# kirilllzaitsev/vision_mtl

Hardware: AMD Instinct MI355X
Metric: images/sec fwd+bwd, basic model 128x256 (higher is better)
Workload: dtype f32

## Files before the change

### include/vmtl.h

```cpp
#ifndef VMTL_H
#define VMTL_H

#ifdef __cplusplus
extern "C" {
#endif

#define VMTL_ACT_NONE 0
#define VMTL_ACT_RELU 1
#define VMTL_ACT_HSWISH 2
#define VMTL_ACT_HSIGMOID 3
#define VMTL_ACT_SIGMOID 4

#define VMTL_PREC_FP32 0
#define VMTL_PREC_BF16 1

const char* vmtl_version(void);
const char* vmtl_last_error_string(void);
int vmtl_reload_env(void);
int vmtl_timestamp(long long* out, void* stream);


int vmtl_conv2d_fwd(const float* x, const float* wp, const float* bias, float* y, float* stats,
                    int B, int H, int W, int Cs, int Ho, int Wo, int ldy, int Nw, int Cout,
                    int KH, int KW, int stride, int pad, int act, int shuffle, void* stream);
int vmtl_conv2d_fwd_p(const float* x, const float* wp, const float* bias, float* y, float* stats,
                      int B, int H, int W, int Cs, int Ho, int Wo, int ldy, int Nw, int Cout,
                      int KH, int KW, int stride, int pad, int act, int shuffle, int precision, void* stream);
int vmtl_conv2d_ksplit(int B, int Ho, int Wo, int ldy, int Ktot);
int vmtl_conv2d_fwd_ws(const float* x, const float* wp, const float* bias, float* y, float* ws, int B, int H, int W, int Cs,
                       int Ho, int Wo, int ldy, int Nw, int Cout, int KH, int KW, int stride, int pad, void* stream);
int vmtl_conv2d_fwd_ws_p(const float* x, const float* wp, const float* bias, float* y, float* ws, int B, int H, int W,
                         int Cs, int Ho, int Wo, int ldy, int Nw, int Cout, int KH, int KW, int stride, int pad,
                         int precision, void* stream);
int vmtl_conv2d_stats_rows(int B, int Ho, int Wo, int ldy);
int vmtl_conv2d_stats_block(int B, int Ho, int Wo, int ldy);

int vmtl_conv1x1_stats_block(int M, int ldy, int Ks, int variant);
int vmtl_conv1x1_stats_rows(int M, int ldy, int Ks, int variant);
int vmtl_conv1x1_fwd(const float* x, const float* wp, const float* bias, float* y, float* stats, int M, int Ks, int ldy,
                     int Nw, int Cout, void* stream);
int vmtl_conv1x1_fwd_p(const float* x, const float* wp, const float* bias, float* y, float* stats, int M, int Ks, int ldy,
                       int Nw, int Cout, int precision, void* stream);
int vmtl_conv1x1_cat_fwd(const float* x, int K1, const float* x2, int K2s, const float* wp, const float* bias, float* y,
                         float* stats, int M, int ldy, int Nw, int Cout, void* stream);
int vmtl_conv1x1_cat_dgrad(const float* dy, const float* wp, float* dx, int N1, float* dx2, int N2s, int N2, int M,
                           int Ks, void* stream);
int vmtl_conv1x1_cat_fwd_p(const float* x, int K1, const float* x2, int K2s, const float* wp, const float* bias, float* y,
                           float* stats, int M, int ldy, int Nw, int Cout, int precision, void* stream);
int vmtl_conv1x1_cat_dgrad_p(const float* dy, const float* wp, float* dx, int N1, float* dx2, int N2s, int N2, int M,
                             int Ks, int precision, void* stream);
int vmtl_conv1x1_cat_wgrad(const float* x, int K1, const float* x2, int K2s, const float* dy, float* slabs, int splits,
                           int M, int ldy, int Nw, void* stream);
int vmtl_conv1x1_cat_wgrad_p(const float* x, int K1, const float* x2, int K2s, const float* dy, float* slabs, int splits,
                             int M, int ldy, int Nw, int precision, void* stream);
int vmtl_conv1x1_bn_fwd(const float* x, const float* coef_a, const float* coef_c, int act_in, float* a_out,
                        const float* wp, const float* bias, float* y, float* stats, int M, int Ks, int ldy, int Nw,
                        int Cout, void* stream);
int vmtl_conv1x1_bnbwd(const float* dy, const float* wp, float* dz, float* stats, const float* ez_x,
                       const float* ez_mean, const float* ez_invstd, const float* ez_gamma, const float* ez_beta,
                       int ez_act, int M, int Ks, int ldy, int Nw, int Cout, void* stream);
int vmtl_conv1x1_bn_fwd_p(const float* x, const float* coef_a, const float* coef_c, int act_in, float* a_out,
                          const float* wp, const float* bias, float* y, float* stats, int M, int Ks, int ldy, int Nw,
                          int Cout, int precision, void* stream);
int vmtl_conv1x1_bnbwd_p(const float* dy, const float* wp, float* dz, float* stats, const float* ez_x,
                         const float* ez_mean, const float* ez_invstd, const float* ez_gamma, const float* ez_beta,
                         int ez_act, int M, int Ks, int ldy, int Nw, int Cout, int precision, void* stream);
int vmtl_conv1x1_bn_res_fwd(const float* x, const float* coef_a, const float* coef_c, int act_in, const float* res,
                            float* a_out, const float* wp, const float* bias, float* y, float* stats, int M, int Ks,
                            int ldy, int Nw, int Cout, void* stream);
int vmtl_conv1x1_bnbwd_add(const float* dy, const float* wp, const float* addend, float* dz, float* stats,
                           const float* ez_x, const float* ez_mean, const float* ez_invstd, const float* ez_gamma,
                           const float* ez_beta, int ez_act, int M, int Ks, int ldy, int Nw, int Cout, void* stream);
int vmtl_conv1x1_bn_res_fwd_p(const float* x, const float* coef_a, const float* coef_c, int act_in, const float* res,
                              float* a_out, const float* wp, const float* bias, float* y, float* stats, int M, int Ks,
                              int ldy, int Nw, int Cout, int precision, void* stream);
int vmtl_conv1x1_bnbwd_add_p(const float* dy, const float* wp, const float* addend, float* dz, float* stats,
                             const float* ez_x, const float* ez_mean, const float* ez_invstd, const float* ez_gamma,
                             const float* ez_beta, int ez_act, int M, int Ks, int ldy, int Nw, int Cout, int precision,
                             void* stream);

int vmtl_conv2d_bnbwd(const float* x, const float* wp, float* y, float* stats, const float* ez_x, const float* ez_mean,
                      const float* ez_invstd, const float* ez_gamma, const float* ez_beta, int ez_act, int B, int H,
                      int W, int Cs, int Ho, int Wo, int ldy, int Nw, int Cout, int KH, int KW, int stride, int pad,
                      void* stream);
int vmtl_conv2d_bnbwd_p(const float* x, const float* wp, float* y, float* stats, const float* ez_x, const float* ez_mean,
                        const float* ez_invstd, const float* ez_gamma, const float* ez_beta, int ez_act, int B, int H,
                        int W, int Cs, int Ho, int Wo, int ldy, int Nw, int Cout, int KH, int KW, int stride, int pad,
                        int precision, void* stream);

int vmtl_conv2d_up2_fwd(const float* xl, const float* skip, const float* wp_eff, float* y, float* stats,
                        int B, int H2, int W2, int C0s, int C1s, int ldy, int Cout, void* stream);
int vmtl_conv2d_up2_fwd_p(const float* xl, const float* skip, const float* wp_eff, float* y, float* stats,
                          int B, int H2, int W2, int C0s, int C1s, int ldy, int Cout, int precision, void* stream);
int vmtl_conv2d_up2_stats_block(int B, int H2, int W2, int ldy);
int vmtl_conv2d_up2_ksplit(int B, int H2, int W2, int ldy, int Ktot);
int vmtl_conv2d_up2_fwd_ws(const float* xl, const float* skip, const float* wp_eff, float* y, float* ws, int B, int H2,
                           int W2, int C0s, int C1s, int ldy, int Cout, void* stream);
int vmtl_conv2d_up2_fwd_ws_p(const float* xl, const float* skip, const float* wp_eff, float* y, float* ws, int B, int H2,
                             int W2, int C0s, int C1s, int ldy, int Cout, int precision, void* stream);
int vmtl_conv2d_up2_halo(const float* xl, const float* skip, const float* wp_eff, float* y, float* stats,
                         int B, int H2, int W2, int C0s, int C1s, int ldy, int Cout, void* stream);
int vmtl_conv2d_up2_halo_supported(int B, int H2, int W2, int C0s, int C1s, int ldy, int Cout);
int vmtl_conv2d_up2_halo_stat_rows(int B, int H2, int W2, int C0s, int C1s, int ldy, int Cout);
int vmtl_conv2d_up2_halo_stat_block(int C0s, int C1s, int ldy, int Cout);
int vmtl_pack_up2_fwd(const float* w, float* dst, int Cout, int C0, int C0s, int C1, int C1s, void* stream);
int vmtl_pack_up2_dgrad(const float* w, float* dst, int Cout, int Cos, int C0, int Cin, void* stream);
int vmtl_unpack_up2(const float* slabs, float* grad, int Cout, int Cos, int C0, int Cin, int nslabs, void* stream);

int vmtl_conv2d_wgrad_splits(int M, int Nw, int Ktot);
int vmtl_conv2d_wgrad(const float* x, const float* dy, float* slabs, int splits, int B, int H, int W, int Cs,
                      int Ho, int Wo, int ldy, int Nw, int KH, int KW, int stride, int pad, void* stream);
int vmtl_conv2d_wgrad_p(const float* x, const float* dy, float* slabs, int splits, int B, int H, int W, int Cs,
                        int Ho, int Wo, int ldy, int Nw, int KH, int KW, int stride, int pad, int precision,
                        void* stream);

int vmtl_conv3x3_wgrad_small_supported(int Cs, int ldy, int W);
int vmtl_conv3x3_wgrad_small_slabs(int B, int H, int W);
int vmtl_conv3x3_wgrad_small(const float* x, const float* dy, float* slabs, int nslabs, int B, int H, int W, int Cs,
                             int ldy, int Nw, void* stream);


int vmtl_conv3x3_small_supported(int Cs, int Nw);
int vmtl_conv3x3_small_tiles(int B, int H, int W);
int vmtl_conv3x3_small_stat_rows(int B, int H, int W);
int vmtl_conv3x3_small_stat_block(int B, int H, int W);
int vmtl_conv3x3_small(const float* x, const float* x2, const float* pa, const float* pb, const float* pc,
                       int act_in, float* a_out, const float* wp, const float* bias, float* y, float* yb, int Ca,
                       float* stats, int ep_mode, const float* ez_x, const float* ez_mean, const float* ez_invstd,
                       const float* ez_gamma, const float* ez_beta, int ez_act, int B, int H, int W, int Cs, int ldy,
                       int Nw, int Cout, void* stream);

int vmtl_conv3x3_halo_supported(int B, int H, int W, int Cs, int ldy, int Nw);
int vmtl_conv3x3_halo_stat_rows(int B, int H, int W);
int vmtl_conv3x3_halo_stat_block(int B, int H, int W);
int vmtl_conv3x3_halo(const float* x, const float* pa, const float* pc, int act_in, float* a_out, const float* wp,
                      const float* bias, float* y, float* stats, int ep_mode, const float* ez_x, const float* ez_mean,
                      const float* ez_invstd, const float* ez_gamma, const float* ez_beta, int ez_act, int B, int H,
                      int W, int Cs, int ldy, int Nw, int Cout, void* stream);

int vmtl_dwconv_fwd(const float* x, const float* wp, float* y, int B, int H, int W, int Cs, int Ho, int Wo,
                    int K, int stride, int pad, void* stream);
int vmtl_dwconv_bn_stats_rows(int M, int Cs);
int vmtl_dwconv_bn_stats_block(int M, int Cs);
int vmtl_dwconv_bn_fwd(const float* x, const float* coef_a, const float* coef_c, int act, const float* wp, float* y,
                       float* a_out, float* partial, int B, int H, int W, int Cs, int Ho, int Wo, int K, int stride,
                       int pad, void* stream);
int vmtl_dwconv_bwd_data(const float* dy, const float* wp, float* dx, int B, int H, int W, int Cs, int Ho,
                         int Wo, int K, int stride, int pad, void* stream);
int vmtl_dwconv_bwd_data_add(const float* dy, const float* wp, const float* addend, float* dx, int B, int H, int W,
                             int Cs, int Ho, int Wo, int K, int stride, int pad, void* stream);
int vmtl_dwconv_bwd_weight_rows(int M, int Cs);
int vmtl_dwconv_bwd_weight(const float* x, const float* dy, float* partial, float* dw, int B, int H, int W,
                           int C, int Cs, int Ho, int Wo, int K, int stride, int pad, void* stream);
#define VMTL_DW_ROUTE_ACT_MASK 3
#define VMTL_DW_ROUTE_SPEC 4
#define VMTL_DW_ROUTE_K5 8
#define VMTL_DW_ROUTE_S2 16
#define VMTL_DW_ROUTE_WLDS 32
#define VMTL_DW_ROUTE_FIN32 64
#define VMTL_DW_ROUTE_QL(r) (1 << (((r) >> 8) & 7))
int vmtl_dwconv_bn_fwd_route(int B, int H, int W, int Cs, int Ho, int Wo, int K, int stride, int pad, int act);
int vmtl_dwconv_bwd_data_route(int B, int H, int W, int Cs, int Ho, int Wo, int K, int stride, int pad);
int vmtl_dwconv_bwd_weight_route(int B, int H, int W, int C, int Cs, int Ho, int Wo, int K, int stride, int pad);

int vmtl_pack_weights(const float* src, float* dst, int R1, int R0, int T, int C, int Cs, long long sr1,
                      long long sr0, long long st, long long sc, int flip, void* stream);
int vmtl_pack_weights_scaled(const float* src, float* dst, int R1, int R0, int T, int C, int Cs, long long sr1,
                             long long sr0, long long st, long long sc, int flip, const float* scale, int sstride,
                             int smode, void* stream);
int vmtl_unpack_weights_stitch(const float* packed, float* grad, const float* w, const float* scale, int sstride,
                               float* ds, float* work, int R0, int T, int C, int Cs, int nslabs, long long slab_stride,
                               int reduce_all, void* stream);
int vmtl_pack_desc_bytes(void);
int vmtl_pack_weights_batch(const void* descs, int n, long long total, void* stream);
int vmtl_pack_weights_slice(const float* src, float* dst, int R0, int T, int C, int group, long long sr0,
                            long long st, long long sc, int flip, void* stream);
int vmtl_unpack_weights(const float* packed, float* grad, int R1, int R0, int T, int C, int Cs,
                        long long sr1, long long sr0, long long st, long long sc, int flip, int nslabs,
                        long long slab_stride, void* stream);

int vmtl_reduce_rows(int M);
int vmtl_bn_stats(const float* x, int M, int C, int Cs, float* partial, int nblk_from_conv,
                  int rows_per_blk_from_conv, float eps, float momentum, float* running_mean, float* running_var, long long* num_batches_tracked,
                  float* save_mean, float* save_invstd, void* stream);
int vmtl_bn_eval_stats(const float* running_mean, const float* running_var, int C, int Cs, float eps,
                       float* save_mean, float* save_invstd, void* stream);
int vmtl_bn_stats_coef(const float* x, int M, int C, int Cs, float* partial, int nblk_from_conv,
                       int rows_per_blk_from_conv, float eps, float momentum, float* running_mean, float* running_var,
                       long long* num_batches_tracked, float* save_mean, float* save_invstd, const float* gamma,
                       const float* beta, float* coef_a, float* coef_c, void* stream);
int vmtl_bn_eval_stats_coef(const float* running_mean, const float* running_var, int C, int Cs, float eps,
                            float* save_mean, float* save_invstd, const float* gamma, const float* beta,
                            float* coef_a, float* coef_c, void* stream);
int vmtl_bn_eval_desc_bytes(void);
int vmtl_bn_eval_stats_batch(const void* descs, int n, int max_cs, void* stream);
int vmtl_bn_apply(const float* x, const float* mean, const float* invstd, const float* gamma,
                  const float* beta, const float* mul, const float* res, float* y, long long M, int C,
                  int Cs, int act, void* stream);
int vmtl_bn_fuse_max_rows(void);
int vmtl_bn_apply_fused(const float* x, const float* partial, int nblk, int rows_per_blk, float eps, float momentum,
                        float* running_mean, float* running_var, long long* num_batches_tracked, float* save_mean,
                        float* save_invstd, const float* gamma, const float* beta, const float* mul, const float* res,
                        float* y, long long M, int C, int Cs, int act, void* stream);
int vmtl_bn_bwd(const float* x, const float* dy, const float* mean, const float* invstd, const float* gamma,
                const float* beta, const float* mul, float* dmul, float* partial, float* sum_dz,
                float* sum_dzx, float* dx, int M, int C, int Cs, int act, int training, void* stream);
int vmtl_bn_bwd_finalize(const float* partial, int nblk, int M, int C, int Cs, float* sum_dz, float* sum_dzx,
                         const float* mean, const float* invstd, const float* gamma, int training, float* coef_a,
                         float* coef_b, float* coef_c, void* stream);
int vmtl_bn_bwd_apply(const float* x, const float* dz, const float* mean, const float* invstd, const float* gamma,
                      const float* sum_dz, const float* sum_dzx, float* dx, int M, int C, int Cs, int training,
                      void* stream);

int vmtl_bn_act_pool2_fwd(const float* x, const float* mean, const float* invstd, const float* gamma,
                          const float* beta, float* y, int B, int H, int W, int C, int Cs, int act, void* stream);
int vmtl_bn_act_pool2_bwd(const float* x, const float* dyp, const float* mean, const float* invstd,
                          const float* gamma, const float* beta, float* partial, float* sum_dz, float* sum_dzx,
                          float* dx, int B, int H, int W, int C, int Cs, int act, int training, void* stream);

int vmtl_conv2d_dgrad_s2_supported(int K, int pad);
long long vmtl_conv2d_dgrad_s2_ws(int B, int H, int W, int Cs, int Ho, int Wo, int ldy, int K, int pad);
long long vmtl_pack_dgrad_s2_size(int Cin, int ldy, int K, int pad);
int vmtl_pack_dgrad_s2(const float* w, float* dst, int Cout, int Cin, int ldy, int K, int pad, void* stream);
int vmtl_conv2d_dgrad_s2(const float* dy, const float* wp, float* dx, float* ws, int B, int H, int W, int Cs, int Ho,
                         int Wo, int ldy, int Cin, int K, int pad, void* stream);
int vmtl_conv2d_dgrad_s2_p(const float* dy, const float* wp, float* dx, float* ws, int B, int H, int W, int Cs, int Ho,
                           int Wo, int ldy, int Cin, int K, int pad, int precision, void* stream);
int vmtl_bn_act_pool3s2_fwd(const float* x, const float* mean, const float* invstd, const float* gamma,
                            const float* beta, float* a_out, float* y, unsigned char* idx, int B, int H, int W, int C,
                            int Cs, int act, void* stream);
int vmtl_bn_act_pool3s2_bwd(const float* x, const float* dskip, const float* dyp, const unsigned char* idx,
                            const float* mean, const float* invstd, const float* gamma, const float* beta, float* dz,
                            float* partial, float* sum_dz, float* sum_dzx, float* dx, int B, int H, int W, int C, int Cs,
                            int act, int training, void* stream);
int vmtl_bn_add_act_fwd(const float* z, const float* mean_a, const float* invstd_a, const float* gamma_a,
                        const float* beta_a, const float* res, const float* zd, const float* mean_b, const float* invstd_b,
                        const float* gamma_b, const float* beta_b, float* y, int M, int C, int Cs, int act, void* stream);
int vmtl_bn_add_act_bwd(const float* z, const float* mean_a, const float* invstd_a, const float* gamma_a,
                        const float* beta_a, const float* res, const float* zd, const float* mean_b, const float* invstd_b,
                        const float* gamma_b, const float* beta_b, const float* dy, float* g, float* partial,
                        float* sum_dz_a, float* sum_dzx_a, float* sum_dz_b, float* sum_dzx_b, float* dz, float* dzd, int M,
                        int C, int Cs, int act, int training, void* stream);

int vmtl_colsum(const float* a, const float* b, int M, int C, int Cs, int mode, int reduce_all,
                float* partial, float* out, void* stream);

int vmtl_concat2(const float* a, int Ha, int Wa, int Ca, int Csa, int upa, int oha, int owa,
                 const float* b, int Hb, int Wb, int Cb, int Csb, int upb, int ohb, int owb, float* y,
                 int B, int H, int W, int Cd, void* stream);
int vmtl_concat2_bwd(const float* dy, float* dx, int B, int H, int W, int Cd, int c_off, int Hs, int Ws,
                     int C, int Cs, int up, int oh, int ow, void* stream);
int vmtl_maxpool2_fwd(const float* x, float* y, int B, int H, int W, int Cs, void* stream);
int vmtl_maxpool2_bwd(const float* x, const float* dy, float* dx, int B, int H, int W, int Cs, void* stream);
int vmtl_bilinear_up2_fwd(const float* x, float* y, int B, int H, int W, int Cs, void* stream);
int vmtl_bilinear_up2_bwd(const float* dy, float* dx, int B, int H, int W, int Cs, void* stream);
int vmtl_spatial_mean(const float* x, float* y, int B, int HW, int Cs, void* stream);
int vmtl_channel_bcast(const float* x, const float* s, float* y, int B, int HW, int Cs, int mode, void* stream);
int vmtl_channel_scale_bwd_s(const float* x, const float* dy, float* ds, int B, int HW, int Cs, void* stream);
int vmtl_fc_max_rows(void);
int vmtl_fc_fwd(const float* a, int a_parts, long long a_part_stride, float a_scale, const float* a_z, int a_act,
                float* a_out, const float* w, const float* bias, float* z, float* y, int M, int K, int N, int lda,
                int ldw, int ldy, int act, void* stream);
int vmtl_fc_wgrad(const float* x, int x_parts, long long x_part_stride, float x_scale, const float* dyo, int dy_parts,
                  long long dy_part_stride, const float* zo, float* dw, float* db, int M, int K, int N, int lda, int ldn,
                  int act, void* stream);
int vmtl_hw_reduce_parts(int B, int HW, int Cs);
int vmtl_hw_reduce(const float* x, const float* y, float* part, int B, int HW, int Cs, void* stream);
int vmtl_channel_scale_add(const float* x, const float* s, const float* t, float t_scale, float* y, int B, int HW,
                           int Cs, void* stream);
int vmtl_se_gate_supported(int B, int C, int R);
// ... 159 lines not shown
```

### vision_mtl_amd/csrc/conv_wgrad_small.hip

```cpp
#include "common.h"

#define WS_SW 32
#define WS_LDP 48
#define WS_XROW ((WS_SW + 2) * WS_LDP)
#define WS_YROW (WS_SW * WS_LDP)

struct WsP {
  const float* x;
  const float* dy;
  float* slabs;
  int B, H, W, Cs, ldy, Nw, Ktot;
  int R;
  int bands, strips;
};

template <int NI, int JW>
__global__ __launch_bounds__(256) void wgrad_small_kernel(WsP p) {
  __shared__ __attribute__((aligned(16))) float Xs[4 * WS_XROW];
  __shared__ __attribute__((aligned(16))) float Ys[2 * WS_YROW];
  const int tid = threadIdx.x;
  const int lane = tid & 63, wn = tid >> 6;
  const int l15 = lane & 15, lq = lane >> 4;

  const int seg = blockIdx.x;
  const int band = seg % p.bands;
  const int t0 = seg / p.bands;
  const int strip = t0 % p.strips, b = t0 / p.strips;
  const int c0 = strip * WS_SW;
  const int r0 = band * p.R, r1 = min(p.H, r0 + p.R);

  for (int i = tid; i < (4 * WS_XROW) / 4; i += 256) reinterpret_cast<f32x4*>(Xs)[i] = (f32x4){0.f, 0.f, 0.f, 0.f};
  for (int i = tid; i < (2 * WS_YROW) / 4; i += 256) reinterpret_cast<f32x4*>(Ys)[i] = (f32x4){0.f, 0.f, 0.f, 0.f};

  const int CQ = p.Cs >> 2, YQ = p.ldy >> 2;
  constexpr unsigned OOB = 0xFFFFFFFFu;
  int xoff[2], xlds[2];
#pragma unroll
  for (int it = 0; it < 2; ++it) {
    const int idx = tid + it * 256;
    const int px = idx / CQ, q = idx - px * CQ;
    const int c = c0 - 1 + px;
    const bool ok = idx < (WS_SW + 2) * CQ && c >= 0 && c < p.W;
    xoff[it] = ok ? (c * p.Cs + q * 4) * 4 : -1;
    xlds[it] = idx < (WS_SW + 2) * CQ ? px * WS_LDP + q * 4 : -1;
  }
  int yoff[2], ylds[2];
#pragma unroll
  for (int it = 0; it < 2; ++it) {
    const int idx = tid + it * 256;
    const int px = idx / YQ, q = idx - px * YQ;
    const bool ok = idx < WS_SW * YQ;
    yoff[it] = ok ? ((c0 + px) * p.ldy + q * 4) * 4 : -1;
    ylds[it] = ok ? px * WS_LDP + q * 4 : -1;
  }
  const __amdgpu_buffer_rsrc_t rs_x =
      buf_rsrc(p.x, (int)((unsigned)p.B * p.H * p.W * p.Cs * 4u));
  const __amdgpu_buffer_rsrc_t rs_dy =
      buf_rsrc(p.dy, (int)((unsigned)p.B * p.H * p.W * p.ldy * 4u));
  auto load_x = [&](int rr, f32x4* rx) {
    const bool rok = rr >= 0 && rr < p.H;
    const unsigned base = (unsigned)(b * p.H + rr) * (unsigned)p.W * (unsigned)p.Cs * 4u;
#pragma unroll
    for (int it = 0; it < 2; ++it) rx[it] = buf_load16(rs_x, (rok & (xoff[it] >= 0)) ? base + (unsigned)xoff[it] : OOB);
  };
  auto load_y = [&](int rr, f32x4* ry) {
    const bool rok = rr < r1;
    const unsigned base = (unsigned)(b * p.H + rr) * (unsigned)p.W * (unsigned)p.ldy * 4u;
#pragma unroll
    for (int it = 0; it < 2; ++it) ry[it] = buf_load16(rs_dy, (rok & (yoff[it] >= 0)) ? base + (unsigned)yoff[it] : OOB);
  };
  auto store_x = [&](int rr, const f32x4* rx) {
    float* xs = Xs + ((rr + 1) & 3) * WS_XROW;
#pragma unroll
    for (int it = 0; it < 2; ++it)
      if (xlds[it] >= 0) *reinterpret_cast<f32x4*>(xs + xlds[it]) = rx[it];
  };
  auto store_y = [&](int buf, const f32x4* ry) {
    float* ys = Ys + buf * WS_YROW;
#pragma unroll
    for (int it = 0; it < 2; ++it)
      if (ylds[it] >= 0) *reinterpret_cast<f32x4*>(ys + ylds[it]) = ry[it];
  };

  int bdh[JW];
  int bcol[JW];
#pragma unroll
  for (int jw = 0; jw < JW; ++jw) {
    const int kk = (wn + 4 * jw) * 16 + l15;
    if (kk < p.Ktot) {
      const int tap = kk / p.Cs, ci = kk - tap * p.Cs;
      const int th = tap / 3;
      bdh[jw] = th - 1;
      bcol[jw] = (lq + tap - 3 * th) * WS_LDP + ci;
    } else {
      bdh[jw] = 0;
      bcol[jw] = lq * WS_LDP + p.Cs;
    }
  }
  const int acol = lq * WS_LDP + l15;

  f32x4 acc[NI][JW];
#pragma unroll
  for (int i = 0; i < NI; ++i)
#pragma unroll
    for (int jw = 0; jw < JW; ++jw) acc[i][jw] = (f32x4){0.f, 0.f, 0.f, 0.f};

  f32x4 rx[2], ry[2];
  __syncthreads();
  load_x(r0 - 1, rx);
  store_x(r0 - 1, rx);
  load_x(r0, rx);
  store_x(r0, rx);
  load_x(r0 + 1, rx);
  store_x(r0 + 1, rx);
  load_y(r0, ry);
  store_y(0, ry);
  __syncthreads();

  for (int r = r0; r < r1; ++r) {
    const int buf = (r - r0) & 1;
    const bool more = r + 1 < r1;
    if (more) {
      load_x(r + 2, rx);
      load_y(r + 1, ry);
    }
    const float* ys = Ys + buf * WS_YROW + acol;
    const float* xb[JW];
#pragma unroll
    for (int jw = 0; jw < JW; ++jw) xb[jw] = Xs + ((r + bdh[jw] + 1) & 3) * WS_XROW + bcol[jw];
#pragma unroll
    for (int s = 0; s < WS_SW / 4; ++s) {
      float fa[NI], fb[JW];
#pragma unroll
      for (int i = 0; i < NI; ++i) fa[i] = ys[4 * s * WS_LDP + i * 16];
#pragma unroll
      for (int jw = 0; jw < JW; ++jw) fb[jw] = xb[jw][4 * s * WS_LDP];
#pragma unroll
      for (int i = 0; i < NI; ++i)
#pragma unroll
        for (int jw = 0; jw < JW; ++jw)
          acc[i][jw] = __builtin_amdgcn_mfma_f32_16x16x4f32(fa[i], fb[jw], acc[i][jw], 0, 0, 0);
    }
    if (more) {
      store_x(r + 2, rx);
      store_y(buf ^ 1, ry);
    }
    __syncthreads();
  }

  float* slab = p.slabs + (size_t)seg * p.Nw * p.Ktot;
#pragma unroll
  for (int i = 0; i < NI; ++i)
#pragma unroll
    for (int jw = 0; jw < JW; ++jw) {
      const int kk = (wn + 4 * jw) * 16 + l15;
#pragma unroll
      for (int e = 0; e < 4; ++e) {
        const int co = i * 16 + 4 * lq + e;
        if (co < p.Nw && kk < p.Ktot) slab[(size_t)co * p.Ktot + kk] = acc[i][jw][e];
      }
    }
}

static void ws_geometry(int B, int H, int W, int* R, int* bands, int* strips) {
  static EnvInt e_target{"VMTL_WS_TARGET", 1024};
  const int st = W / WS_SW;
  long long nb = cdivll((long long)env_int(e_target), (long long)B * st);
  if (nb < 1) nb = 1;
  int rows = cdiv(H, (int)nb);
  if (rows < 8) rows = H < 8 ? H : 8;
  *R = rows;
  *bands = cdiv(H, rows);
  *strips = st;
}

extern "C" int vmtl_conv3x3_wgrad_small_supported(int Cs, int ldy, int W) {
  static EnvInt e{"VMTL_WGRAD_SMALL", 1};
  return env_int(e) != 0 && Cs >= 4 && Cs <= 36 && !(Cs & 3) && ldy >= 4 && ldy <= 36 && !(ldy & 3) && !(Cs > 32 && ldy > 32) &&
         W >= WS_SW && W % WS_SW == 0;
}

extern "C" int vmtl_conv3x3_wgrad_small_slabs(int B, int H, int W) {
  if (B <= 0 || H <= 0 || W < WS_SW || W % WS_SW) return 0;
  int R, bands, strips;
  ws_geometry(B, H, W, &R, &bands, &strips);
  return B * strips * bands;
}

template <int NI>
static int ws_launch(const WsP& p, int jwn, int grid, hipStream_t st) {
  switch (jwn) {
    case 1: hipLaunchKernelGGL((wgrad_small_kernel<NI, 1>), dim3(grid), dim3(256), 0, st, p); break;
    case 2: hipLaunchKernelGGL((wgrad_small_kernel<NI, 2>), dim3(grid), dim3(256), 0, st, p); break;
    case 3: hipLaunchKernelGGL((wgrad_small_kernel<NI, 3>), dim3(grid), dim3(256), 0, st, p); break;
    case 4: hipLaunchKernelGGL((wgrad_small_kernel<NI, 4>), dim3(grid), dim3(256), 0, st, p); break;
    case 5: hipLaunchKernelGGL((wgrad_small_kernel<NI, 5>), dim3(grid), dim3(256), 0, st, p); break;
    case 6: hipLaunchKernelGGL((wgrad_small_kernel<NI, 6>), dim3(grid), dim3(256), 0, st, p); break;
    default: return VMTL_ERR_UNSUPPORTED;
  }
  return vmtl_check_launch();
}

extern "C" int vmtl_conv3x3_wgrad_small(const float* x, const float* dy, float* slabs, int nslabs, int B, int H, int W, int Cs,
                                        int ldy, int Nw, void* stream) {
  VMTL_ENTER();
  if (!x || !dy || !slabs || B <= 0 || H <= 0 || Nw <= 0 || Nw > ldy) return VMTL_ERR_ARG;
  if (!vmtl_conv3x3_wgrad_small_supported(Cs, ldy, W)) return VMTL_ERR_UNSUPPORTED;
  if ((long long)B * H * W * Cs * 4 >= (1ll << 32) || (long long)B * H * W * ldy * 4 >= (1ll << 32)) return VMTL_ERR_UNSUPPORTED;
  WsP p;
  p.x = x; p.dy = dy; p.slabs = slabs; p.B = B; p.H = H; p.W = W; p.Cs = Cs; p.ldy = ldy; p.Nw = Nw; p.Ktot = 9 * Cs;
  ws_geometry(B, H, W, &p.R, &p.bands, &p.strips);
  const int grid = B * p.strips * p.bands;
  if (nslabs != grid) return VMTL_ERR_ARG;
  const int nj = cdiv(p.Ktot, 16), jwn = cdiv(nj, 4);
  hipStream_t st = (hipStream_t)stream;
  switch (cdiv(Nw, 16)) {
    case 1: return ws_launch<1>(p, jwn, grid, st);
    case 2: return ws_launch<2>(p, jwn, grid, st);
    case 3: return ws_launch<3>(p, jwn, grid, st);
    default: return VMTL_ERR_UNSUPPORTED;
  }
}
```

### vision_mtl_amd/ops.py

```python
from __future__ import annotations

import contextlib
import functools
import math
import os
import struct
import weakref
from typing import NamedTuple

import torch

from ._lib import lib
from .precision import conv_prec_code, pw_prec_code

ACT_NONE, ACT_RELU, ACT_HSWISH, ACT_HSIGMOID, ACT_SIGMOID = 0, 1, 2, 3, 4
ACT_CODES = {None: 0, "none": 0, "relu": 1, "hardswish": 2, "hardsigmoid": 3, "sigmoid": 4}


def ceil4(c: int) -> int:
    return (c + 3) // 4 * 4


def _stream() -> int:
    return torch.cuda.current_stream().cuda_stream
# ... 349 lines not shown
        self.epoch += 1
        if self.dirty:
            if capturing:
                return
            self._build_table()
        if self.table is not None:
            table, n, total = self.table
            _k("vmtl_pack_weights_batch", descs=table, n=n, total=total)
        for e in self.live:
            w = e["wref"]()
            if w is not None:
                e["version"], e["epoch"] = w._version, self.epoch
                if "sref" in e:
                    sw = e["sref"]()
                    if sw is not None and e.get("sver") is not None:
                        e["sver"] = (sw.data_ptr(), sw._version) + tuple(e["sver"][2:])
        if self.custom or self.table_side is not None:
            use_side = side.enabled and not side.task_mode
            if use_side:
                main = torch.cuda.current_stream()
                s = side.stream(main.device)
                s.wait_stream(main)
                ctx = torch.cuda.stream(s)
            else:
                ctx = contextlib.nullcontext()
            with ctx:
                if self.table_side is not None:
                    table, n, total = self.table_side
                    _k("vmtl_pack_weights_batch", descs=table, n=n, total=total)
                for e in self.custom.values():
                    w = e["wref"]()
                    if w is None:
                        continue
                    deps = [d() for d in e.get("deps", ())]
                    if any(d is None for d in deps):
                        continue
                    e["fn"](w, e["dst"])
                    e["version"] = (w._version,) + tuple((d.data_ptr(), d._version) for d in deps)
                    e["epoch"] = self.epoch
                if use_side:
                    ev = torch.cuda.Event()
                    ev.record()
                    self.custom_ready = ev


packs = _PackCache()


class _EvalBNTable:

    DESC = "<QQQQQQQQiifi"

    def __init__(self):
        self.tables = weakref.WeakKeyDictionary()
        self.active = None

    @staticmethod
    def _layers(model):
        return [m for m in model.modules() if isinstance(m, torch.nn.BatchNorm2d) and not m.training
                and m.running_mean is not None]

    @staticmethod
    def _signature(layers):
        ptr = lambda t: 0 if t is None else t.data_ptr()
        return tuple((id(m), m.running_mean.data_ptr(), m.running_var.data_ptr(), ptr(m.weight), ptr(m.bias),
                      m.num_features, float(m.eps)) for m in layers)

    def table(self, model):
        import struct

        layers = self._layers(model)
        if not layers:
            return None
        sig = self._signature(layers)
        t = self.tables.get(model)
        if t is not None and t["sig"] == sig:
            return t
        if torch.cuda.is_current_stream_capturing():
            raise RuntimeError("eval_bn_table: the BatchNorm table of this model must be built before the capture "
                               "(enter eval_bn_table once eagerly, e.g. in a warm-up step)")
        dev = layers[0].running_mean.device
        sizes = [ceil4(m.num_features) for m in layers]
        buf = torch.zeros(4 * sum(sizes), dtype=torch.float32, device=dev)
        recs, lookup, off = [], {}, 0
        for m, Cs in zip(layers, sizes):
            _req(m.running_mean, "running_mean"), _req(m.running_var, "running_var")
            mean, invstd, ca, cc = (buf[off + i * Cs: off + (i + 1) * Cs] for i in range(4))
            off += 4 * Cs
            g = 0 if m.weight is None else m.weight.data_ptr()
            b = 0 if m.bias is None else m.bias.data_ptr()
            recs.append(struct.pack(self.DESC, m.running_mean.data_ptr(), m.running_var.data_ptr(), g, b,
                                    mean.data_ptr(), invstd.data_ptr(), ca.data_ptr(), cc.data_ptr(), m.num_features,
                                    Cs, float(m.eps), 0))
            lookup[m.running_mean.data_ptr()] = (mean, invstd, ca, cc, m.num_features, float(m.eps), g, b)
        size = lib().raw("vmtl_bn_eval_desc_bytes")()
        blob = b"".join(r.ljust(size, b"\0") for r in recs)
        t = {"sig": sig, "descs": torch.frombuffer(bytearray(blob), dtype=torch.uint8).to(dev), "n": len(recs),
             "max_cs": max(sizes), "buf": buf, "lookup": lookup}
        self.tables[model] = t
        return t

    def get(self, rm, C, eps, coef=None):
        if self.active is None:
            return None
        e = self.active.get(rm.data_ptr())
        if e is None or e[4] != C or e[5] != float(eps):
            return None
        if coef is not None and tuple(0 if t is None else t.data_ptr() for t in coef) != e[6:8]:
            return None
        return e[:4]


eval_bn = _EvalBNTable()


@contextlib.contextmanager
def eval_bn_table(model):
    t = eval_bn.table(model)
    prev = eval_bn.active
    if t is not None:
        _k("vmtl_bn_eval_stats_batch", descs=t["descs"], n=t["n"], max_cs=t["max_cs"])
        eval_bn.active = t["lookup"] if prev is None else {**prev, **t["lookup"]}
    try:
        yield t
    finally:
        eval_bn.active = prev


def _bn_eval_stats(rm, rv, C, Cs, eps, like):
    e = eval_bn.get(rm, C, eps)
    if e is not None:
        return e[0], e[1]
    mean, invstd = _empty((Cs,), like), _empty((Cs,), like)
    _k("vmtl_bn_eval_stats", running_mean=rm, running_var=rv, C=C, Cs=Cs, eps=eps, save_mean=mean, save_invstd=invstd)
    return mean, invstd


def pack(src, R1, R0, T, C, Cs, sr1, sr0, st, sc, flip=0, out=None):
    dst = _empty((R1 * R0, T * Cs), src) if out is None else out
    _k("vmtl_pack_weights", src=src, dst=dst, R1=R1, R0=R0, T=T, C=C, Cs=Cs, sr1=sr1, sr0=sr0, st=st, sc=sc, flip=flip)
    return dst


def unpack(packed, layout, out, nslabs=1, slab_stride=0):
    R1, R0, T, C, Cs, sr1, sr0, st, sc, flip = layout
    _k("vmtl_unpack_weights", packed=packed, grad=out, R1=R1, R0=R0, T=T, C=C, Cs=Cs, sr1=sr1, sr0=sr0, st=st,
       sc=sc, flip=flip, nslabs=nslabs, slab_stride=slab_stride)
    return out


def _wgrad(x, dy, g, *, Nw, flop, xflop=None, prec=0):
    B, H, W, Cs, Ho, Wo, ldy, KH, KW, stride, pad = g
    if (KH == 3 and KW == 3 and stride == 1 and pad == 1 and B * H * W * max(Cs, ldy) * 4 < 1 << 32
            and lib().raw("vmtl_conv3x3_wgrad_small_supported")(Cs, ldy, W)):
        ns = lib().raw("vmtl_conv3x3_wgrad_small_slabs")(B, H, W)
        slabs = _empty((ns, Nw, 9 * Cs), x)
        _k("vmtl_conv3x3_wgrad_small", _flop=flop, _xflop=xflop, x=x, dy=dy, slabs=slabs, nslabs=ns, B=B, H=H, W=W, Cs=Cs, ldy=ldy,
           Nw=Nw)
        return slabs, ns
    splits = lib().raw("vmtl_conv2d_wgrad_splits")(B * Ho * Wo, Nw, KH * KW * Cs)
    slabs = _empty((splits, Nw, KH * KW * Cs), x)
    _kp("vmtl_conv2d_wgrad", prec, _flop=flop, _xflop=xflop, x=x, dy=dy, slabs=slabs, splits=splits, B=B, H=H, W=W, Cs=Cs, Ho=Ho, Wo=Wo,
       ldy=ldy, Nw=Nw, KH=KH, KW=KW, stride=stride, pad=pad)
    return slabs, splits


def _colsum(a, b, M, C, Cs, mode=0, reduce_all=0, out=None):
    partial = _empty((_reduce_rows(M) + 1, Cs), a)
    if out is None:
        out = _empty((1 if reduce_all else C,), a)
    _k("vmtl_colsum", a=a, b=b, M=M, C=C, Cs=Cs, mode=mode, reduce_all=reduce_all, partial=partial, out=out)
    return out


def _wgrad_into(x, dy, g, layout, dw, flop, prec=0):
    slabs, ns = _wgrad(x, dy, g, Nw=layout.R1 * layout.R0, flop=flop, prec=prec)
    unpack(slabs, layout, dw, nslabs=ns)


def _wgrad_two_heads(x, dy, g, lay_a, lay_b, wa, wb, slots, flop, prec):
    swa, sba, swb, sbb = slots
    Ca, Cb, row = lay_a.R0, lay_b.R0, lay_a.T * lay_a.Cs
    N = Ca + Cb
    slabs, ns = _wgrad(x, dy, g, Nw=N, flop=flop, prec=prec)
    dwa, dwb = _grad_buf(wa.shape, swa, x), _grad_buf(wb.shape, swb, x)
    unpack(slabs, lay_a, dwa, nslabs=ns, slab_stride=N * row)
    unpack(slabs.view(-1)[Ca * row:], lay_b, dwb, nslabs=ns, slab_stride=N * row)
    db = _colsum(dy, None, g.M, N, g.ldy)
    dba, dbb = _grad_buf((Ca,), sba, x), _grad_buf((Cb,), sbb, x)
    _copy_vec(db, dba, Ca)
    _copy_vec(db[Ca:], dbb, Cb)
    return _grad_ret(dwa, swa), _grad_ret(dba, sba), _grad_ret(dwb, swb), _grad_ret(dbb, sbb)


def _bias_grad(bias, slot, dy, M, Cout, ldy, zero, fork):
    arena = getattr(bias, "_vmtl_arena", None) if slot is not None else None
    if zero:
        if slot is None:
            db = _empty((Cout,), dy)
            _k("vmtl_fill_zero", p=db, n=Cout)
            return db
        capturing = torch.cuda.is_current_stream_capturing()
        if arena is None or id(bias) not in arena._zero_bias or (capturing and side.enabled and not side.task_mode):
            with side.branch(True, M, fork, dy):
                _k("vmtl_fill_zero", p=slot, n=Cout)
            if arena is not None and not capturing:
                arena._zero_bias.add(id(bias))
        return None
    with side.branch(slot is not None, M, fork, dy):
        db = _colsum(dy, None, M, Cout, ldy, out=slot)
    if slot is not None:
        if arena is not None:
            arena._zero_bias.discard(id(bias))
        return None
    return db


FUSE_DW = os.environ.get("VMTL_FUSE_DW", "1") != "0"
_PW = os.environ.get("VMTL_PW", "1") != "0"
_PW_MAX_ROWS = int(os.environ.get("VMTL_PW_MAX_ROWS", str(1 << 21)))
_SMALL_MIN_ROWS = int(os.environ.get("VMTL_SMALL_MIN_ROWS", str(1 << 16)))
_SMALL_STATS = os.environ.get("VMTL_SMALL_STATS", "1") != "0"
_MID_HALO = os.environ.get("VMTL_MID_HALO", "1") != "0"
_MID_HALO_MIN_ROWS = int(os.environ.get("VMTL_MID_HALO_MIN_ROWS", str(1 << 16)))
_UP2_HALO = os.environ.get("VMTL_UP2_HALO", "1") != "0"


class ConvPlan(NamedTuple):
    route: str
    ksplit: int
    stats_rows: int
    rpb: int


def conv_plan(B, H, W, Cs, Ho, Wo, ldy, KH, KW, stride, pad, shuffle=0, prec=0, epilogue=None) -> ConvPlan:
    raw = lib().raw
    M = B * Ho * Wo
    pw = _PW and KH == 1 and KW == 1 and stride == 1 and pad == 0 and not shuffle and M <= _PW_MAX_ROWS
    ks = 1 if shuffle or pw else raw("vmtl_conv2d_ksplit")(B, Ho, Wo, ldy, KH * KW * Cs)
    if ks > 1 or (epilogue == "bnbwd" and os.environ.get("VMTL_BNBWD_FUSE", "1") == "0"):
        epilogue = None
    tap3 = KH == 3 and KW == 3 and stride == 1 and pad == 1 and not shuffle
    if pw:
        route = "pw"
    elif (tap3 and ldy <= 36 and M >= _SMALL_MIN_ROWS and M * 36 <= 0x7FFFFFFF
          and conv3x3_small_supported(Cs, ldy) and (not epilogue or (_SMALL_STATS and Ho % 4 == 0 and Wo % 32 == 0))):
        route = "small"
    elif (_MID_HALO and prec == 0 and tap3 and M >= _MID_HALO_MIN_ROWS and ks == 1
          and raw("vmtl_conv3x3_halo_supported")(B, Ho, Wo, Cs, ldy, ldy)
          and (not epilogue or raw("vmtl_conv3x3_halo_stat_rows")(B, Ho, Wo) > 0)):
        route = "mid_halo"
    else:
        route = "ksplit" if ks > 1 else "igemm"
    if not epilogue:
        return ConvPlan(route, ks, 0, 0)
    if route == "small":
        rows, rpb = raw("vmtl_conv3x3_small_stat_rows")(B, Ho, Wo), raw("vmtl_conv3x3_small_stat_block")(B, Ho, Wo)
    elif route == "mid_halo":
        rows, rpb = raw("vmtl_conv3x3_halo_stat_rows")(B, Ho, Wo), raw("vmtl_conv3x3_halo_stat_block")(B, Ho, Wo)
    elif route == "pw":
        rows, rpb = raw("vmtl_conv1x1_stats_rows")(M, ldy, Cs, 0), raw("vmtl_conv1x1_stats_block")(M, ldy, Cs, 0)
    else:
        rows, rpb = raw("vmtl_conv2d_stats_rows")(B, Ho, Wo, ldy), raw("vmtl_conv2d_stats_block")(B, Ho, Wo, ldy)
    return ConvPlan(route, ks, rows, rpb)


def up2_plan(B, H2, W2, C0s, C1s, ldy, Cout, prec, want_stats) -> ConvPlan:
    raw = lib().raw
    ks = raw("vmtl_conv2d_up2_ksplit")(B, H2, W2, ldy, 4 * C0s + 9 * C1s)
    rows = rpb = 0
    if _UP2_HALO and prec == 0 and ks == 1 and raw("vmtl_conv2d_up2_halo_supported")(B, H2, W2, C0s, C1s, ldy, Cout):
        route = "up2_halo"
        if want_stats:
            rows = raw("vmtl_conv2d_up2_halo_stat_rows")(B, H2, W2, C0s, C1s, ldy, Cout)
            rpb = raw("vmtl_conv2d_up2_halo_stat_block")(C0s, C1s, ldy, Cout) if rows else 0
    elif ks > 1:
        route = "ksplit"
    else:
        route = "igemm"
        if want_stats:
            bm, Mq = raw("vmtl_conv2d_up2_stats_block")(B, H2, W2, ldy), B * H2 * W2
            if Mq % bm == 0:
                rows, rpb = 4 * (Mq // bm), bm
    return ConvPlan(route, ks, rows, rpb)


def _mid_halo(x, wp, y, B, H, W, Cs, ldy, Nw, Cout, flop, pa=None, pc=None, act_in=ACT_NONE, a_out=None, bias=None,
              stats=None, ep_mode=0, ez=None):
    ez = ez or (None, None, None, None, None, ACT_NONE)
    _k("vmtl_conv3x3_halo", _flop=flop, x=x, pa=pa, pc=pc, act_in=act_in, a_out=a_out, wp=wp, bias=bias, y=y, stats=stats,
       ep_mode=ep_mode, ez_x=ez[0], ez_mean=ez[1], ez_invstd=ez[2], ez_gamma=ez[3], ez_beta=ez[4], ez_act=ez[5], B=B, H=H,
       W=W, Cs=Cs, ldy=ldy, Nw=Nw, Cout=Cout)


def _halo_launch(route, x, wp, y, g, Nw, Cout, flop, **kw):
    (_small if route == "small" else _mid_halo)(x, wp, y, g.B, g.H, g.W, g.Cs, g.ldy, Nw, Cout, flop, **kw)


def _conv_launch(x, wp, bias, y, g, *legacy, Cout=None, Nw=None, shuffle=0, cin=None, algo_flop=None, prec=0, plan=None, stats=None,
                 pw_prec=0):
    if legacy:
        B, H, W, Cs, Ho, Wo, ldy, Nw, Cout, KH, KW, stride, pad = (g, *legacy)
        g = ConvGeom(B, H, W, Cs, Ho, Wo, ldy, KH, KW, stride, pad)
    B, H, W, Cs, Ho, Wo, ldy, KH, KW, stride, pad = g
    if Nw is None:
        Nw = Cout
    if plan is None:
        plan = conv_plan(B, H, W, Cs, Ho, Wo, ldy, KH, KW, stride, pad, shuffle, prec)
# ... 2613 lines not shown
```

Before: 2730.

## Extend small 3x3 wgrad kernel to wider channels with tail rows and 8-wave blocks

Generalises the LDS-staged small-channel 3x3 weight-gradient kernel with template parameters for LDS row pitch, wave count and a scalar tail for output channels past a multiple of 16. Layers with up to 68 input or output channels, and odd counts such as 17 or 33, can now use this path instead of the generic split-K wgrad. The per-shape grid target also changes so wider channels get fewer bands. A pixel-count threshold and an FP32-only check gate the wide path, which adds more template instantiations and register pressure on the 8-wave variants.

Result: faster. 2758, median of 6 (+1.0%).

```diff
diff --git a/include/vmtl.h b/include/vmtl.h
--- a/include/vmtl.h
+++ b/include/vmtl.h
@@ -115,7 +115,9 @@
                         void* stream);
 
 int vmtl_conv3x3_wgrad_small_supported(int Cs, int ldy, int W);
+int vmtl_conv3x3_wgrad_small_supported_p(int Cs, int ldy, int W, long long pixels, int precision);
 int vmtl_conv3x3_wgrad_small_slabs(int B, int H, int W);
+int vmtl_conv3x3_wgrad_small_slabs_for(int B, int H, int W, int Cs, int ldy, int Nw);
 int vmtl_conv3x3_wgrad_small(const float* x, const float* dy, float* slabs, int nslabs, int B, int H, int W, int Cs,
                              int ldy, int Nw, void* stream);
 
diff --git a/vision_mtl_amd/csrc/conv_wgrad_small.hip b/vision_mtl_amd/csrc/conv_wgrad_small.hip
--- a/vision_mtl_amd/csrc/conv_wgrad_small.hip
+++ b/vision_mtl_amd/csrc/conv_wgrad_small.hip
@@ -1,9 +1,8 @@
 #include "common.h"
 
 #define WS_SW 32
-#define WS_LDP 48
-#define WS_XROW ((WS_SW + 2) * WS_LDP)
-#define WS_YROW (WS_SW * WS_LDP)
+#define WS_NARROW 36
+#define WS_MAXC 68
 
 struct WsP {
   const float* x;
@@ -14,10 +13,19 @@
   int bands, strips;
 };
 
-template <int NI, int JW>
-__global__ __launch_bounds__(256) void wgrad_small_kernel(WsP p) {
-  __shared__ __attribute__((aligned(16))) float Xs[4 * WS_XROW];
-  __shared__ __attribute__((aligned(16))) float Ys[2 * WS_YROW];
+template <int NI, int JW, int NTR, int NW, int LDX, int LDY>
+__global__ __launch_bounds__(NW * 64) void wgrad_small_kernel(WsP p) {
+  constexpr int NT = NW * 64;
+  constexpr int XROW = (WS_SW + 2) * LDX;
+  constexpr int YROW = WS_SW * LDY;
+  constexpr int XIT = ((WS_SW + 2) * ((LDX == 48 ? WS_NARROW : WS_MAXC) / 4) + NT - 1) / NT;
+  constexpr int YIT = (WS_SW * ((LDY == 48 ? WS_NARROW : WS_MAXC) / 4) + NT - 1) / NT;
+  static_assert(LDX % 32 == 16 && LDY % 32 == 16, "the four quarters of a fragment read start 16 banks apart");
+  static_assert((LDX == 48 ? WS_NARROW : WS_MAXC) < LDX, "a dead lane reads the zero pad float at channel Cs");
+  static_assert(NI * 16 + NTR <= LDY, "every co tile (and the tail quad) lies inside a dY pixel");
+  static_assert(NTR >= 0 && NTR <= 4, "the tail is one 16-byte LDS word");
+  __shared__ __attribute__((aligned(16))) float Xs[4 * XROW];
+  __shared__ __attribute__((aligned(16))) float Ys[2 * YROW];
   const int tid = threadIdx.x;
   const int lane = tid & 63, wn = tid >> 6;
   const int l15 = lane & 15, lq = lane >> 4;
@@ -29,29 +37,29 @@
   const int c0 = strip * WS_SW;
   const int r0 = band * p.R, r1 = min(p.H, r0 + p.R);
 
-  for (int i = tid; i < (4 * WS_XROW) / 4; i += 256) reinterpret_cast<f32x4*>(Xs)[i] = (f32x4){0.f, 0.f, 0.f, 0.f};
-  for (int i = tid; i < (2 * WS_YROW) / 4; i += 256) reinterpret_cast<f32x4*>(Ys)[i] = (f32x4){0.f, 0.f, 0.f, 0.f};
+  for (int i = tid; i < (4 * XROW) / 4; i += NT) reinterpret_cast<f32x4*>(Xs)[i] = (f32x4){0.f, 0.f, 0.f, 0.f};
+  for (int i = tid; i < (2 * YROW) / 4; i += NT) reinterpret_cast<f32x4*>(Ys)[i] = (f32x4){0.f, 0.f, 0.f, 0.f};
 
   const int CQ = p.Cs >> 2, YQ = p.ldy >> 2;
   constexpr unsigned OOB = 0xFFFFFFFFu;
-  int xoff[2], xlds[2];
-#pragma unroll
-  for (int it = 0; it < 2; ++it) {
-    const int idx = tid + it * 256;
+  int xoff[XIT], xlds[XIT];
+#pragma unroll
+  for (int it = 0; it < XIT; ++it) {
+    const int idx = tid + it * NT;
     const int px = idx / CQ, q = idx - px * CQ;
     const int c = c0 - 1 + px;
     const bool ok = idx < (WS_SW + 2) * CQ && c >= 0 && c < p.W;
     xoff[it] = ok ? (c * p.Cs + q * 4) * 4 : -1;
-    xlds[it] = idx < (WS_SW + 2) * CQ ? px * WS_LDP + q * 4 : -1;
-  }
-  int yoff[2], ylds[2];
-#pragma unroll
-  for (int it = 0; it < 2; ++it) {
-    const int idx = tid + it * 256;
+    xlds[it] = idx < (WS_SW + 2) * CQ ? px * LDX + q * 4 : -1;
+  }
+  int yoff[YIT], ylds[YIT];
+#pragma unroll
+  for (int it = 0; it < YIT; ++it) {
+    const int idx = tid + it * NT;
     const int px = idx / YQ, q = idx - px * YQ;
     const bool ok = idx < WS_SW * YQ;
     yoff[it] = ok ? ((c0 + px) * p.ldy + q * 4) * 4 : -1;
-    ylds[it] = ok ? px * WS_LDP + q * 4 : -1;
+    ylds[it] = ok ? px * LDY + q * 4 : -1;
   }
   const __amdgpu_buffer_rsrc_t rs_x =
       buf_rsrc(p.x, (int)((unsigned)p.B * p.H * p.W * p.Cs * 4u));
@@ -61,24 +69,24 @@
     const bool rok = rr >= 0 && rr < p.H;
     const unsigned base = (unsigned)(b * p.H + rr) * (unsigned)p.W * (unsigned)p.Cs * 4u;
 #pragma unroll
-    for (int it = 0; it < 2; ++it) rx[it] = buf_load16(rs_x, (rok & (xoff[it] >= 0)) ? base + (unsigned)xoff[it] : OOB);
+    for (int it = 0; it < XIT; ++it) rx[it] = buf_load16(rs_x, (rok & (xoff[it] >= 0)) ? base + (unsigned)xoff[it] : OOB);
   };
   auto load_y = [&](int rr, f32x4* ry) {
     const bool rok = rr < r1;
     const unsigned base = (unsigned)(b * p.H + rr) * (unsigned)p.W * (unsigned)p.ldy * 4u;
 #pragma unroll
-    for (int it = 0; it < 2; ++it) ry[it] = buf_load16(rs_dy, (rok & (yoff[it] >= 0)) ? base + (unsigned)yoff[it] : OOB);
+    for (int it = 0; it < YIT; ++it) ry[it] = buf_load16(rs_dy, (rok & (yoff[it] >= 0)) ? base + (unsigned)yoff[it] : OOB);
   };
   auto store_x = [&](int rr, const f32x4* rx) {
-    float* xs = Xs + ((rr + 1) & 3) * WS_XROW;
-#pragma unroll
-    for (int it = 0; it < 2; ++it)
+    float* xs = Xs + ((rr + 1) & 3) * XROW;
+#pragma unroll
+    for (int it = 0; it < XIT; ++it)
       if (xlds[it] >= 0) *reinterpret_cast<f32x4*>(xs + xlds[it]) = rx[it];
   };
   auto store_y = [&](int buf, const f32x4* ry) {
-    float* ys = Ys + buf * WS_YROW;
-#pragma unroll
-    for (int it = 0; it < 2; ++it)
+    float* ys = Ys + buf * YROW;
+#pragma unroll
+    for (int it = 0; it < YIT; ++it)
       if (ylds[it] >= 0) *reinterpret_cast<f32x4*>(ys + ylds[it]) = ry[it];
   };
 
@@ -86,26 +94,31 @@
   int bcol[JW];
 #pragma unroll
   for (int jw = 0; jw < JW; ++jw) {
-    const int kk = (wn + 4 * jw) * 16 + l15;
+    const int kk = (wn + NW * jw) * 16 + l15;
     if (kk < p.Ktot) {
       const int tap = kk / p.Cs, ci = kk - tap * p.Cs;
       const int th = tap / 3;
       bdh[jw] = th - 1;
-      bcol[jw] = (lq + tap - 3 * th) * WS_LDP + ci;
+      bcol[jw] = (lq + tap - 3 * th) * LDX + ci;
     } else {
       bdh[jw] = 0;
-      bcol[jw] = lq * WS_LDP + p.Cs;
-    }
-  }
-  const int acol = lq * WS_LDP + l15;
+      bcol[jw] = lq * LDX + p.Cs;
+    }
+  }
+  const int acol = lq * LDY + l15;
 
   f32x4 acc[NI][JW];
 #pragma unroll
   for (int i = 0; i < NI; ++i)
 #pragma unroll
     for (int jw = 0; jw < JW; ++jw) acc[i][jw] = (f32x4){0.f, 0.f, 0.f, 0.f};
-
-  f32x4 rx[2], ry[2];
+  float tacc[NTR > 0 ? NTR : 1][JW];
+#pragma unroll
+  for (int t = 0; t < (NTR > 0 ? NTR : 1); ++t)
+#pragma unroll
+    for (int jw = 0; jw < JW; ++jw) tacc[t][jw] = 0.f;
+
+  f32x4 rx[XIT], ry[YIT];
   __syncthreads();
   load_x(r0 - 1, rx);
   store_x(r0 - 1, rx);
@@ -124,22 +137,32 @@
       load_x(r + 2, rx);
       load_y(r + 1, ry);
     }
-    const float* ys = Ys + buf * WS_YROW + acol;
+    const float* ys = Ys + buf * YROW + acol;
     const float* xb[JW];
 #pragma unroll
-    for (int jw = 0; jw < JW; ++jw) xb[jw] = Xs + ((r + bdh[jw] + 1) & 3) * WS_XROW + bcol[jw];
+    for (int jw = 0; jw < JW; ++jw) xb[jw] = Xs + ((r + bdh[jw] + 1) & 3) * XROW + bcol[jw];
 #pragma unroll
     for (int s = 0; s < WS_SW / 4; ++s) {
       float fa[NI], fb[JW];
 #pragma unroll
-      for (int i = 0; i < NI; ++i) fa[i] = ys[4 * s * WS_LDP + i * 16];
-#pragma unroll
-      for (int jw = 0; jw < JW; ++jw) fb[jw] = xb[jw][4 * s * WS_LDP];
+      for (int i = 0; i < NI; ++i) fa[i] = ys[4 * s * LDY + i * 16];
+#pragma unroll
+      for (int jw = 0; jw < JW; ++jw) fb[jw] = xb[jw][4 * s * LDX];
 #pragma unroll
       for (int i = 0; i < NI; ++i)
 #pragma unroll
         for (int jw = 0; jw < JW; ++jw)
           acc[i][jw] = __builtin_amdgcn_mfma_f32_16x16x4f32(fa[i], fb[jw], acc[i][jw], 0, 0, 0);
+      if (NTR > 0) {
+        const float* yt = Ys + buf * YROW + (4 * s + lq) * LDY + NI * 16;
+        f32x4 ty;
+        if constexpr (NTR == 1) ty[0] = yt[0];
+        else ty = *reinterpret_cast<const f32x4*>(yt);
+#pragma unroll
+        for (int t = 0; t < NTR; ++t)
+#pragma unroll
+          for (int jw = 0; jw < JW; ++jw) tacc[t][jw] += ty[t] * fb[jw];
+      }
     }
     if (more) {
       store_x(r + 2, rx);
@@ -153,19 +176,35 @@
   for (int i = 0; i < NI; ++i)
 #pragma unroll
     for (int jw = 0; jw < JW; ++jw) {
-      const int kk = (wn + 4 * jw) * 16 + l15;
+      const int kk = (wn + NW * jw) * 16 + l15;
 #pragma unroll
       for (int e = 0; e < 4; ++e) {
         const int co = i * 16 + 4 * lq + e;
         if (co < p.Nw && kk < p.Ktot) slab[(size_t)co * p.Ktot + kk] = acc[i][jw][e];
       }
     }
-}
-
-static void ws_geometry(int B, int H, int W, int* R, int* bands, int* strips) {
-  static EnvInt e_target{"VMTL_WS_TARGET", 1024};
+  if (NTR > 0) {
+#pragma unroll
+    for (int t = 0; t < NTR; ++t)
+#pragma unroll
+      for (int jw = 0; jw < JW; ++jw) {
+        const float v = quarter_sum(tacc[t][jw]);
+        const int co = NI * 16 + t;
+        const int kk = (wn + NW * jw) * 16 + l15;
+        if (lq == 0 && co < p.Nw && kk < p.Ktot) slab[(size_t)co * p.Ktot + kk] = v;
+      }
+  }
+}
+
+static EnvInt ws_e_wide{"VMTL_WGRAD_SMALL_WIDE", 1};
+
+static bool ws_before_tails(int Cs, int ldy) { return Cs <= WS_NARROW && ldy <= WS_NARROW && !(Cs > 32 && ldy > 32); }
+
+static void ws_geometry(int B, int H, int W, int Cs, int ldy, int* R, int* bands, int* strips) {
+  static EnvInt e_target{"VMTL_WS_TARGET", 0};
   const int st = W / WS_SW;
-  long long nb = cdivll((long long)env_int(e_target), (long long)B * st);
+  const int target = env_int(e_target) > 0 ? env_int(e_target) : Cs > WS_NARROW ? 256 : ldy > WS_NARROW ? 512 : 1024;
+  long long nb = cdivll((long long)target, (long long)B * st);
   if (nb < 1) nb = 1;
   int rows = cdiv(H, (int)nb);
   if (rows < 8) rows = H < 8 ? H : 8;
@@ -176,29 +215,67 @@
 
 extern "C" int vmtl_conv3x3_wgrad_small_supported(int Cs, int ldy, int W) {
   static EnvInt e{"VMTL_WGRAD_SMALL", 1};
-  return env_int(e) != 0 && Cs >= 4 && Cs <= 36 && !(Cs & 3) && ldy >= 4 && ldy <= 36 && !(ldy & 3) && !(Cs > 32 && ldy > 32) &&
-         W >= WS_SW && W % WS_SW == 0;
+  if (env_int(e) == 0 || Cs < 4 || (Cs & 3) || ldy < 4 || (ldy & 3) || W < WS_SW || W % WS_SW) return 0;
+  if (ws_before_tails(Cs, ldy)) return 1;
+  return env_int(ws_e_wide) != 0 && Cs <= WS_MAXC && ldy <= WS_MAXC;
+}
+
+extern "C" int vmtl_conv3x3_wgrad_small_supported_p(int Cs, int ldy, int W, long long pixels, int precision) {
+  static EnvInt e_min{"VMTL_WS_WIDE_MIN_PIXELS", 65536};
+  if (!vmtl_conv3x3_wgrad_small_supported(Cs, ldy, W)) return 0;
+  if (ws_before_tails(Cs, ldy)) return 1;
+  return precision == VMTL_PREC_FP32 && pixels >= env_int(e_min);
+}
+
+extern "C" int vmtl_conv3x3_wgrad_small_slabs_for(int B, int H, int W, int Cs, int ldy, int Nw) {
+  if (B <= 0 || H <= 0 || W < WS_SW || W % WS_SW || Cs <= 0 || ldy <= 0 || Nw <= 0) return 0;
+  int R, bands, strips;
+  ws_geometry(B, H, W, Cs, ldy, &R, &bands, &strips);
+  return B * strips * bands;
 }
 
 extern "C" int vmtl_conv3x3_wgrad_small_slabs(int B, int H, int W) {
-  if (B <= 0 || H <= 0 || W < WS_SW || W % WS_SW) return 0;
-  int R, bands, strips;
-  ws_geometry(B, H, W, &R, &bands, &strips);
-  return B * strips * bands;
-}
-
-template <int NI>
+  return vmtl_conv3x3_wgrad_small_slabs_for(B, H, W, WS_NARROW, WS_NARROW, WS_NARROW);
+}
+
+template <int NI, int NTR, int NW, int LDX, int LDY>
 static int ws_launch(const WsP& p, int jwn, int grid, hipStream_t st) {
-  switch (jwn) {
-    case 1: hipLaunchKernelGGL((wgrad_small_kernel<NI, 1>), dim3(grid), dim3(256), 0, st, p); break;
-    case 2: hipLaunchKernelGGL((wgrad_small_kernel<NI, 2>), dim3(grid), dim3(256), 0, st, p); break;
-    case 3: hipLaunchKernelGGL((wgrad_small_kernel<NI, 3>), dim3(grid), dim3(256), 0, st, p); break;
-    case 4: hipLaunchKernelGGL((wgrad_small_kernel<NI, 4>), dim3(grid), dim3(256), 0, st, p); break;
-    case 5: hipLaunchKernelGGL((wgrad_small_kernel<NI, 5>), dim3(grid), dim3(256), 0, st, p); break;
-    case 6: hipLaunchKernelGGL((wgrad_small_kernel<NI, 6>), dim3(grid), dim3(256), 0, st, p); break;
-    default: return VMTL_ERR_UNSUPPORTED;
-  }
+#define WS_CASE(J)                                                                                                       \
+  case J: hipLaunchKernelGGL((wgrad_small_kernel<NI, J, NTR, NW, LDX, LDY>), dim3(grid), dim3(NW * 64), 0, st, p); break;
+  if constexpr (LDX == 48) {
+    switch (jwn) {
+      WS_CASE(1) WS_CASE(2) WS_CASE(3) WS_CASE(4) WS_CASE(5) WS_CASE(6)
+      default: return VMTL_ERR_UNSUPPORTED;
+    }
+  } else {
+    switch (jwn) {
+      WS_CASE(3) WS_CASE(4) WS_CASE(5)
+      default: return VMTL_ERR_UNSUPPORTED;
+    }
+  }
+#undef WS_CASE
   return vmtl_check_launch();
+}
+
+template <int NW, int LDX, int LDY>
+static int ws_launch_rows(const WsP& p, bool tail, int jwn, int grid, hipStream_t st) {
+  const int full = p.Nw >> 4, rest = p.Nw & 15;
+  if constexpr (LDY == 48) {
+    if (tail && rest == 1 && full == 1) return ws_launch<1, 1, NW, LDX, LDY>(p, jwn, grid, st);
+    if (tail && rest == 1 && full == 2) return ws_launch<2, 1, NW, LDX, LDY>(p, jwn, grid, st);
+    if (tail && rest >= 2 && rest <= 4 && full == 1) return ws_launch<1, 4, NW, LDX, LDY>(p, jwn, grid, st);
+    if (tail && rest >= 2 && rest <= 4 && full == 2) return ws_launch<2, 4, NW, LDX, LDY>(p, jwn, grid, st);
+    switch (cdiv(p.Nw, 16)) {
+      case 1: return ws_launch<1, 0, NW, LDX, LDY>(p, jwn, grid, st);
+      case 2: return ws_launch<2, 0, NW, LDX, LDY>(p, jwn, grid, st);
+      case 3: return ws_launch<3, 0, NW, LDX, LDY>(p, jwn, grid, st);
+      default: return VMTL_ERR_UNSUPPORTED;
+    }
+  } else {
+    if (p.Nw > 64) return ws_launch<4, 4, NW, LDX, LDY>(p, jwn, grid, st);
+    if (p.Nw > 48) return ws_launch<4, 0, NW, LDX, LDY>(p, jwn, grid, st);
+    return ws_launch<3, 0, NW, LDX, LDY>(p, jwn, grid, st);
+  }
 }
 
 extern "C" int vmtl_conv3x3_wgrad_small(const float* x, const float* dy, float* slabs, int nslabs, int B, int H, int W, int Cs,
@@ -209,15 +286,15 @@
   if ((long long)B * H * W * Cs * 4 >= (1ll << 32) || (long long)B * H * W * ldy * 4 >= (1ll << 32)) return VMTL_ERR_UNSUPPORTED;
   WsP p;
   p.x = x; p.dy = dy; p.slabs = slabs; p.B = B; p.H = H; p.W = W; p.Cs = Cs; p.ldy = ldy; p.Nw = Nw; p.Ktot = 9 * Cs;
-  ws_geometry(B, H, W, &p.R, &p.bands, &p.strips);
+  ws_geometry(B, H, W, Cs, ldy, &p.R, &p.bands, &p.strips);
   const int grid = B * p.strips * p.bands;
   if (nslabs != grid) return VMTL_ERR_ARG;
-  const int nj = cdiv(p.Ktot, 16), jwn = cdiv(nj, 4);
+  const bool tail = env_int(ws_e_wide) != 0;
+  const int nj = cdiv(p.Ktot, 16);
   hipStream_t st = (hipStream_t)stream;
-  switch (cdiv(Nw, 16)) {
-    case 1: return ws_launch<1>(p, jwn, grid, st);
-    case 2: return ws_launch<2>(p, jwn, grid, st);
-    case 3: return ws_launch<3>(p, jwn, grid, st);
-    default: return VMTL_ERR_UNSUPPORTED;
-  }
-}
+  if (Cs <= WS_NARROW)
+    return ldy <= WS_NARROW ? ws_launch_rows<4, 48, 48>(p, tail, cdiv(nj, 4), grid, st)
+                            : ws_launch_rows<4, 48, 80>(p, tail, cdiv(nj, 4), grid, st);
+  return ldy <= WS_NARROW ? ws_launch_rows<8, 80, 48>(p, tail, cdiv(nj, 8), grid, st)
+                          : ws_launch_rows<8, 80, 80>(p, tail, cdiv(nj, 8), grid, st);
+}
diff --git a/vision_mtl_amd/ops.py b/vision_mtl_amd/ops.py
--- a/vision_mtl_amd/ops.py
+++ b/vision_mtl_amd/ops.py
@@ -525,8 +525,8 @@
 def _wgrad(x, dy, g, *, Nw, flop, xflop=None, prec=0):
     B, H, W, Cs, Ho, Wo, ldy, KH, KW, stride, pad = g
     if (KH == 3 and KW == 3 and stride == 1 and pad == 1 and B * H * W * max(Cs, ldy) * 4 < 1 << 32
-            and lib().raw("vmtl_conv3x3_wgrad_small_supported")(Cs, ldy, W)):
-        ns = lib().raw("vmtl_conv3x3_wgrad_small_slabs")(B, H, W)
+            and lib().raw("vmtl_conv3x3_wgrad_small_supported_p")(Cs, ldy, W, B * H * W, prec)):
+        ns = lib().raw("vmtl_conv3x3_wgrad_small_slabs_for")(B, H, W, Cs, ldy, Nw)
         slabs = _empty((ns, Nw, 9 * Cs), x)
         _k("vmtl_conv3x3_wgrad_small", _flop=flop, _xflop=xflop, x=x, dy=dy, slabs=slabs, nslabs=ns, B=B, H=H, W=W, Cs=Cs, ldy=ldy,
            Nw=Nw)
```
